# aleksandrina-streltsova/lidar-global-registration

Hardware: AMD Instinct MI355X
Metric: scan-pair registrations/sec (higher is better)
Workload: dtype f32

## Files before the change

### lidar-global-registration_amd/csrc/lgr_match.hip

```cpp
#include <rocprim/device/device_radix_sort.hpp>
#include <rocprim/device/device_scan.hpp>

#include <algorithm>
#include <vector>

#include "lgr_internal.h"

#include "lgr_match_common.cuh"
#include "lgr_match_cluster.cuh"
#include "lgr_match_pack.cuh"
#include "lgr_match_mfma.cuh"
#include "lgr_match_sweep.cuh"
#include "lgr_match_bounds.cuh"
#include "lgr_match_rerank.cuh"

extern "C" int lgr_match_last_stats(lgr_ctx* ctx, unsigned* out6) {
    if (!ctx || !out6) return LGR_ERR_INVALID_ARG;
    const lgr_match_stats& s = ctx->mstats;
    out6[0] = s.items_ab; out6[1] = s.dense_ab; out6[2] = s.items_ba;
    out6[3] = s.dense_ba; out6[4] = (unsigned) s.sub_cols; out6[5] = (unsigned) s.rg_rows;
    return LGR_OK;
}
extern "C" int lgr_match_last_work(lgr_ctx* ctx, double* executed_fraction) {
    if (!ctx || !executed_fraction) return LGR_ERR_INVALID_ARG;
// ... 136 lines not shown
struct MatchPrep {
    bool armed = false;
    const float* d_a = nullptr;
    int ma = 0, mb = 0;
    bool both = false;
    lgr_match_options mopt{};
    int sub = 1, rg_rows = BLOCK_ROWS, ns = 0;
    float *cen = nullptr, *cen2 = nullptr, *smp = nullptr, *basis = nullptr;
    int* smp_ok = nullptr;
    IrrRef* irr = nullptr;
    bool basis_ready = false;
    Side A;
};
static void match_prep_free(void* p) { delete (MatchPrep*) p; }
static MatchPrep* match_prep_of(lgr_ctx* ctx) {
    if (!ctx->match_prep) { ctx->match_prep = new MatchPrep(); ctx->match_prep_free = match_prep_free; }
    return (MatchPrep*) ctx->match_prep;
}

static int match_cluster(lgr_ctx* ctx, const float* d_a, int ma, const float* d_b, int mb, bool both, bool basis_side_by_side, MatchPrep* P) {
    const lgr_match_options& mo = ctx->mopt;
    int sub = 1;
    while (sub < SUBMAX && (long long) KCL * sub * 1024 < std::max(ma, mb)) sub *= 2;
    if (mo.leaves > 0) sub = mo.leaves;
    sub = std::min(SUBMAX, std::max(1, sub));
    const int n_leaves = KCL * sub;
    const int ns = 2 * KM_SAMPLE;
    char* misc;
    Carve carve{8192};
    const size_t o_cen2 = carve((size_t) MAXLEAF * 33 * 4);
    const size_t o_smp = carve((size_t) ns * 33 * 4), o_ok = carve((size_t) ns * 4), o_label = carve((size_t) ns * 4);
    const size_t o_cbuf = carve((size_t) 2 * KCL * 33 * 4), o_basis = carve((size_t) (34 * 33 + 64) * 4);
    const size_t o_skeys = carve((size_t) 2 * ns * 4), o_svals = carve((size_t) ns * 4), o_sidx = carve((size_t) ns * 4), o_coff = carve(256);
    const size_t o_zero = carve.off;
    const size_t o_kmax = carve(256), o_irr = carve(sizeof(IrrRef)), o_acc1 = carve((size_t) KM_ITERS * KCL * sizeof(KmAcc)), o_acc2 = carve((size_t) MAXLEAF * sizeof(KmAcc));
    const size_t zero_bytes = carve.off - o_zero;
    LGR_TRY(lgr_ws_t(ctx, WS_MATCH_MISC, carve.off, &misc));
    float* cen = (float*) (misc + 256);
    float* cen2 = (float*) (misc + o_cen2);
    float* smp = (float*) (misc + o_smp);
    int* smp_ok = (int*) (misc + o_ok);
    int* label = (int*) (misc + o_label);
    float* cbuf = (float*) (misc + o_cbuf);
    float* basis = (float*) (misc + o_basis);
    unsigned* skeys = (unsigned*) (misc + o_skeys);
    int* svals = (int*) (misc + o_svals);
    int* sidx = (int*) (misc + o_sidx);
    int* coff = (int*) (misc + o_coff);
    unsigned* kmax = (unsigned*) (misc + o_kmax);
    KmAcc* acc1 = (KmAcc*) (misc + o_acc1);
    KmAcc* acc2 = (KmAcc*) (misc + o_acc2);
    LGR_HIP(ctx, hipMemsetAsync(misc + o_zero, 0, zero_bytes, ctx->stream));
    IrrRef* irr = mo.irregular_rows ? (IrrRef*) (misc + o_irr) : nullptr;
    if (irr) km_consensus<<<cdiv(ns, 256), 256, 0, ctx->stream>>>(d_a, ma, d_b, mb, KM_SAMPLE, irr);
    km_sample<<<cdiv(ns, 256), 256, 0, ctx->stream>>>(d_a, ma, d_b, mb, KM_SAMPLE, smp, smp_ok, kmax, irr);
    auto lloyd = [&](lgr_ctx* cx) -> int {
        km_init<<<1, 64, 0, cx->stream>>>(smp, smp_ok, ns, cbuf);
        for (int it = 0; it <= KM_ITERS; ++it) {
            const bool last = it == KM_ITERS;
            km1_step<<<cdiv(ns, KM1_THREADS), KM1_THREADS, 0, cx->stream>>>(smp, smp_ok, ns, kmax, cbuf + (it & 1) * KCL * 33, it ? acc1 + (size_t) (it - 1) * KCL : nullptr,
                                                                            last ? nullptr : acc1 + (size_t) it * KCL, last ? cen : cbuf + ((it + 1) & 1) * KCL * 33, label);
        }
        km_label_keys<<<cdiv(ns, 256), 256, 0, cx->stream>>>(label, ns, skeys, svals);
        LGR_TRY(lgr_sort_pairs_u32(cx, skeys, skeys + ns, svals, sidx, (size_t) ns, 0, 5));
        km_cluster_offsets<<<1, 64, 0, cx->stream>>>(skeys + ns, ns, coff);
        km2_init<<<KCL, 64, 0, cx->stream>>>(smp, sidx, coff, cen, sub, cen2);
        if (sub > 1) {
            for (int it = 0; it < KM2_ITERS; ++it) {
                km2_step<<<dim3(KM2_PIECES, KCL), KM2_THREADS, 0, cx->stream>>>(smp, sidx, coff, kmax, cen2, sub, acc2);
                km2_finalize<<<n_leaves, 64, 0, cx->stream>>>(acc2, kmax, cen2);
            }
        }
        LGR_HIP(cx, hipGetLastError());
        return LGR_OK;
    };
    const bool want_basis = mo.box_bounds != 0;
    if (want_basis && basis_side_by_side) {
        LGR_TRY(lgr_run_pair(ctx, lloyd, [&](lgr_ctx* cx) { return box_basis(cx, mo.box_bounds == 2, smp, smp_ok, ns, basis, []() { return (int) LGR_OK; }); }));
    } else if (want_basis) {
        LGR_TRY(box_basis(ctx, mo.box_bounds == 2, smp, smp_ok, ns, basis, [&]() { return lloyd(ctx); }));
    } else {
        LGR_TRY(lloyd(ctx));
    }
    auto pick_group = [](size_t q_count, size_t t_count) {
        int g = 1024;
        while (g < 4096 && (t_count / g + 1) * q_count * 4 > ((size_t) 6 << 30)) g *= 2;
        return g;
    };
    int rg_rows = both ? pick_group((size_t) mb, (size_t) ma) : BLOCK_ROWS;
    if (ma <= 65536) rg_rows = BLOCK_ROWS;
    P->d_a = d_a; P->ma = ma; P->mb = mb; P->both = both; P->mopt = mo;
    P->sub = sub; P->rg_rows = rg_rows; P->ns = ns;
    P->cen = cen; P->cen2 = cen2; P->smp = smp; P->smp_ok = smp_ok; P->basis = basis; P->basis_ready = want_basis; P->irr = irr;
    return LGR_OK;
}

int lgr_match_prepare(lgr_ctx* ctx, const float* d_a, int ma, int mb, bool both) {
    MatchPrep* P = match_prep_of(ctx);
    P->armed = false;
    if (!d_a || ma <= 0 || mb <= 0) return LGR_OK;
    LGR_HIP(ctx, hipSetDevice(ctx->device));
    LGR_TRY(match_cluster(ctx, d_a, ma, nullptr, mb, both, false, P));
    P->armed = true;
    return LGR_OK;
}
void lgr_match_prepare_cancel(lgr_ctx* ctx) {
    if (ctx && ctx->match_prep) ((MatchPrep*) ctx->match_prep)->armed = false;
// ... 283 lines not shown
    if (f16 && env_int("LGR_MATCH_DEBUG", 0))
        fprintf(stderr, "[lgr] operand statistics: max |x - c|^2 %.6g, dropped energy %.6g (A %.6g, B %.6g) -> %s; irregular rows %d + %d\n", (double) r2, (double) drop2,
                (double) A.nstat_drop, (double) B.nstat_drop, os.rot ? "rotated" : "plain", A.n_irr, B.n_irr);
    st.f16 = f16 ? (os.rot ? 2 : 1) : 0;
    KS = !f16 ? OpFmt<FMT_F32>::KS : os.rot ? OpFmt<FMT_F16R>::KS : OpFmt<FMT_F16>::KS;
    NF = !f16 ? OpFmt<FMT_F32>::NF : os.rot ? OpFmt<FMT_F16R>::NF : OpFmt<FMT_F16>::NF;
    const size_t frag_bytes = f16 ? sizeof(f16x8) : sizeof(float);
    const size_t a_op_bytes = (size_t) ta * NF * 64 * frag_bytes;
    bset_stride = (size_t) tb * NF * 64;
    LGR_TRY(lgr_ws_t(ctx, WS_MATCH_ROWMIN, a_op_bytes + 256, &Aop));
    const size_t b_op_bytes = KCL * bset_stride * frag_bytes;
    LGR_TRY(lgr_ws_t(ctx, WS_MATCH_COLMIN, b_op_bytes + 256, &Bop));
    n_rg = cdiv(ma_pad, rg_rows);
    return LGR_OK;
}

int MatchCall::upload_group_tables() {
    std::vector<int> h_group_start, h_tiles(2 * (size_t) tb);
    int group_cols = GROUP_COLS;
    while (group_cols < 65536 && ((size_t) mb_pad / group_cols + n_leaves) * (size_t) ma_pad * 4 > ((size_t) 24 << 30)) group_cols *= 2;
    for (int l = 0; l < n_leaves; ++l)
        for (int s0 = B.h_leaf_start[l]; s0 < B.h_leaf_start[l + 1]; s0 += group_cols) {
            int s1 = std::min(B.h_leaf_start[l + 1], s0 + group_cols), g = (int) h_group_start.size();
            h_group_start.push_back(s0);
            for (int t = s0 / TILE; t < s1 / TILE; ++t) { h_tiles[t] = g; h_tiles[tb + t] = l; }
        }
    n_groups = (int) h_group_start.size();
    st.sub_cols = n_groups;
    h_group_start.push_back(mb_pad);
    LGR_TRY(lgr_ws_t(ctx, WS_MATCH_BEST_B, (size_t) KCL * n_groups + 2 * (size_t) n_rg + 2 * (size_t) tb + 2 * (size_t) n_groups + n_leaves + 72, &gmaxB));
    gmaxA = gmaxB + (size_t) KCL * n_groups;
    cl_of_rg = (int*) (gmaxA + n_rg);
    tile_group = cl_of_rg + n_rg;
    tile_leaf = tile_group + tb;
    group_start = tile_leaf + tb;
    group_leaf = group_start + n_groups + 1;
    leaf_g0 = group_leaf + n_groups;
    std::vector<int> h(n_rg), hgl(n_groups), hl(n_leaves + 1, n_groups);
    for (int g = 0; g < n_rg; ++g) h[g] = A.h_blkcl[(size_t) g * (rg_rows / BLOCK_ROWS)];
    for (int g = 0; g < n_groups; ++g) hgl[g] = h_tiles[tb + h_group_start[g] / TILE];
    for (int g = n_groups - 1; g >= 0; --g) hl[hgl[g]] = g;
    for (int l = n_leaves - 1; l >= 0; --l) hl[l] = std::min(hl[l], hl[l + 1]);
    LGR_HIP(ctx, hipMemcpyAsync(cl_of_rg, h.data(), h.size() * 4, hipMemcpyHostToDevice, ctx->stream));
    LGR_HIP(ctx, hipMemcpyAsync(tile_group, h_tiles.data(), h_tiles.size() * 4, hipMemcpyHostToDevice, ctx->stream));
    LGR_HIP(ctx, hipMemcpyAsync(group_start, h_group_start.data(), h_group_start.size() * 4, hipMemcpyHostToDevice, ctx->stream));
    LGR_HIP(ctx, hipMemcpyAsync(group_leaf, hgl.data(), hgl.size() * 4, hipMemcpyHostToDevice, ctx->stream));
    LGR_HIP(ctx, hipMemcpyAsync(leaf_g0, hl.data(), hl.size() * 4, hipMemcpyHostToDevice, ctx->stream));
    LGR_HIP(ctx, hipStreamSynchronize(ctx->stream));
    return LGR_OK;
}

static void launch_pack16(bool rot, hipStream_t s, const float* X, const int* perm, int n_pad, int role, const float* cen, const int* blkcl, const F16Scale& sc,
                          void* op, float* nrm, float2* shell) {
    if (rot) pack16_kernel<true><<<cdiv(n_pad, 256), 256, 0, s>>>(X, perm, n_pad, role, cen, blkcl, sc, (_Float16*) op, nrm, shell);
    else pack16_kernel<false><<<cdiv(n_pad, 256), 256, 0, s>>>(X, perm, n_pad, role, cen, blkcl, sc, (_Float16*) op, nrm, shell);
}

PruneWs MatchCall::carve_prune_ws(char* base) const {
    Carve carve{0, base};
    PruneWs w{};
    const size_t n_pairs = (size_t) n_rb * n_leaves;
    w.LBsq = carve.take<float>(n_pairs * 4);
    w.done = carve.take<uint8_t>(n_pairs);
    w.sched = carve.take<uint8_t>(n_pairs);
    w.touched = carve.take<uint8_t>(n_pairs);
    w.mask = carve.take<unsigned>((size_t) n_rb * n_cc * 4);
    w.mask_acc = carve.take<unsigned>((size_t) n_rb * n_cc * 4);
    w.u_rb = carve.take<float>((size_t) n_rb * 4);
    w.u_rt = carve.take<float>((size_t) n_rb * (BLOCK_ROWS / TILE) * 4);
    w.u_leaf = carve.take<unsigned>((size_t) MAXLEAF * 4);
    w.stats = carve.take<MaskStats>(sizeof(MaskStats));
    w.lb_part = carve.take<uint2>((size_t) n_rb * sizeof(uint2));
    w.leaf_first = carve.take<int>((size_t) MAXLEAF * 4);
    w.leaf_last = carve.take<int>((size_t) MAXLEAF * 4);
    w.mask_chk = carve.take<unsigned>(mo.self_check ? (size_t) 2 * n_rb * n_cc * 4 + 256 : 0);
    w.u_stage = carve.take<unsigned>((size_t) n_stage_total * 4);
    w.u_ct = carve.take<unsigned>((size_t) tb * 4);
    w.comp_r = carve.take<uint8_t>((size_t) n_rb * n_groups);
    w.comp_c = carve.take<uint8_t>((size_t) n_leaves * n_rg);
    w.smaxB = carve.take<float>((size_t) KCL * n_stage_total * 4);
    w.coarse_cnt = carve.take<unsigned long long>(32);
    w.u_row = carve.take<float>((size_t) ma_pad * 4);
    w.u_colv = carve.take<float>((size_t) mb_pad * 4);
    w.stage_shell = carve.take<float2>((size_t) KCL * n_stage_total * 8);
    w.rb_shell = carve.take<float2>((size_t) n_rb * 8);
    w.cperm = carve.take<int>((size_t) (n_leaves + TILE) * 4);
    w.cnrm = carve.take<float>((size_t) KCL * (n_leaves + TILE) * 4);
    w.cop = carve.take<f16x8>((size_t) KCL * ((n_leaves + TILE) / TILE) * 7 * 64 * sizeof(f16x8));
    w.clear_begin = (char*) w.done; w.clear_end = (char*) w.comp_r;
    w.bytes = carve.off;
    return w;
}
int MatchCall::prepare_prune_ws() {
    hipStream_t s3 = ctx->stream;
    if (f16) LGR_TRY(lgr_ctx_stream3(ctx, &s3));
    sB.start(ctx, s3, ctx->ev3, s3 != ctx->stream);
    n_cc = cdiv(mb_pad, CHUNK_COLS);
    n_cpad = pad_to(n_leaves, TILE);
    cset_stride = (size_t) (n_cpad / TILE) * NF * 64;
    if (!prune) return LGR_OK;
    char* pb;
    LGR_TRY(lgr_ws_t(ctx, WS_MATCH_PRUNE, carve_prune_ws(nullptr).bytes, &pb));
    W = carve_prune_ws(pb);
    LGR_TRY(sB.fork(ctx->ev[31]));
    LGR_HIP(ctx, hipMemsetAsync(W.clear_begin, 0, W.clear_end - W.clear_begin, sB.s));
    if (f16) {
        centre_perm_kernel<<<cdiv(n_cpad, 256), 256, 0, sB.s>>>(n_leaves, n_cpad, W.cperm);
        launch_pack16(os.rot, sB.s, cen2, W.cperm, n_cpad, 1, cen, nullptr, os.sc, W.cop, W.cnrm, nullptr);
// ... 424 lines not shown
```

### lidar-global-registration_amd/csrc/lgr_match_cluster.cuh

```cuda
#pragma once
#include "lgr_match_common.cuh"

namespace {

struct KmAcc { long long sum[33]; long long cnt; };
__device__ __forceinline__ double km_scale(unsigned kmax_bits) {
    return kmax_bits ? ldexp(1.0, 40 - ((int) (kmax_bits >> 23) - 127)) : 1.0;
}
constexpr int IRR_CAND = 16;
constexpr int IRR_CAP = 1024;
struct IrrRef { double s[3]; double tol; int enabled; int best; unsigned n_ok; unsigned agree[IRR_CAND]; };
__device__ __forceinline__ void block_sums(const float* v, double& s0, double& s1, double& s2) {
    s0 = 0.0; s1 = 0.0; s2 = 0.0;
#pragma unroll
    for (int k = 0; k < 11; ++k) { s0 += (double) v[k]; s1 += (double) v[11 + k]; s2 += (double) v[22 + k]; }
}
__device__ __forceinline__ bool sums_agree(double a0, double a1, double a2, double r0, double r1, double r2, double tol) {
    return fabs(a0 - r0) <= tol && fabs(a1 - r1) <= tol && fabs(a2 - r2) <= tol;
}
__device__ __forceinline__ double sums_tol(double r0, double r1, double r2) { return 1e-5 * fmax(fmax(fabs(r0), fabs(r1)), fabs(r2)); }
__device__ __forceinline__ const float* sample_row(int s, const float* __restrict__ A, int ma, const float* __restrict__ B, int mb, int per_side) {
    const bool fromA = !B || s < per_side;
    const float* X = fromA ? A : B;
    const int m = fromA ? ma : mb;
    if (m <= 0) return nullptr;
    const int t = fromA ? s : s - per_side;
    const long long i = (long long) t * m / (B ? per_side : 2 * per_side);
    return X + (size_t) i * 33;
}
__device__ __forceinline__ bool irr_decide(const IrrRef* __restrict__ ref, int& best) {
    unsigned top = 0u;
    best = 0;
    for (int c = 0; c < IRR_CAND; ++c) { const unsigned a = ref->agree[c]; if (a > top) { top = a; best = c; } }
    const unsigned n_ok = ref->n_ok;
    return n_ok >= 256u && (unsigned long long) top * 1000ull >= (unsigned long long) n_ok * 995ull;
}
__global__ __launch_bounds__(256) void km_consensus(const float* __restrict__ A, int ma, const float* __restrict__ B, int mb, int per_side, IrrRef* __restrict__ ref) {
    __shared__ double cs[IRR_CAND][3];
    __shared__ int cok[IRR_CAND];
    const int ns = 2 * per_side;
    if (threadIdx.x < IRR_CAND) {
        const float* r = sample_row((int) ((long long) threadIdx.x * ns / IRR_CAND), A, ma, B, mb, per_side);
        float v[33];
        const bool ok = r && row_finite(r, v);
        double s0 = 0.0, s1 = 0.0, s2 = 0.0;
        if (ok) block_sums(v, s0, s1, s2);
        cs[threadIdx.x][0] = s0; cs[threadIdx.x][1] = s1; cs[threadIdx.x][2] = s2;
        cok[threadIdx.x] = ok ? 1 : 0;
    }
    __syncthreads();
    const int s = blockIdx.x * blockDim.x + threadIdx.x;
    bool ok = false;
    double s0 = 0.0, s1 = 0.0, s2 = 0.0;
    if (s < ns) {
        const float* r = sample_row(s, A, ma, B, mb, per_side);
        float v[33];
        ok = r && row_finite(r, v);
        if (ok) block_sums(v, s0, s1, s2);
    }
    const int lane = threadIdx.x & 63;
    for (int c = 0; c < IRR_CAND; ++c) {
        const bool a = ok && cok[c] && sums_agree(s0, s1, s2, cs[c][0], cs[c][1], cs[c][2], sums_tol(cs[c][0], cs[c][1], cs[c][2]));
        const int n = __popcll(__ballot(a));
        if (lane == 0 && n) atomicAdd(&ref->agree[c], (unsigned) n);
    }
    const int n_ok = __popcll(__ballot(ok));
    if (lane == 0 && n_ok) atomicAdd(&ref->n_ok, (unsigned) n_ok);
}
__global__ void km_sample(const float* __restrict__ A, int ma, const float* __restrict__ B, int mb, int per_side,
                          float* __restrict__ smp, int* __restrict__ smp_ok, unsigned* __restrict__ kmax , IrrRef* __restrict__ irr_ref) {
    int s = blockIdx.x * blockDim.x + threadIdx.x;
    if (s >= 2 * per_side) return;
    const float* r = sample_row(s, A, ma, B, mb, per_side);
    float v[33];
    bool ok = r && row_finite(r, v);
    if (irr_ref) {
        int best;
        const bool on = irr_decide(irr_ref, best);
        double r0 = 0.0, r1 = 0.0, r2 = 0.0;
        if (on) {
            const float* rr = sample_row((int) ((long long) best * (2 * per_side) / IRR_CAND), A, ma, B, mb, per_side);
            float w[33];
            (void) row_finite(rr, w);
            block_sums(w, r0, r1, r2);
            if (ok) {
                double s0, s1, s2;
                block_sums(v, s0, s1, s2);
                ok = sums_agree(s0, s1, s2, r0, r1, r2, sums_tol(r0, r1, r2));
            }
        }
        if (s == 0) { irr_ref->s[0] = r0; irr_ref->s[1] = r1; irr_ref->s[2] = r2; irr_ref->tol = sums_tol(r0, r1, r2); irr_ref->best = best; irr_ref->enabled = on ? 1 : 0; }
    }
    float mx = 0.f;
    for (int k = 0; k < 33; ++k) { smp[(size_t) s * 33 + k] = ok ? v[k] : 0.f; if (ok) mx = fmaxf(mx, fabsf(v[k])); }
    smp_ok[s] = ok ? 1 : 0;
    for (int o = 32; o > 0; o >>= 1) mx = fmaxf(mx, __shfl_xor(mx, o));
    if ((threadIdx.x & 63) == 0 && mx > 0.f) atomicMax(kmax, __float_as_uint(mx));
}
__global__ void km_init(const float* __restrict__ smp, const int* __restrict__ smp_ok, int ns, float* __restrict__ cen) {
    int c = threadIdx.x;
    if (c >= KCL) return;
    int s = (int) ((long long) c * ns / KCL);
    int tries = 0;
    while (!smp_ok[s] && tries < ns) { s = (s + 1) % ns; ++tries; }
    for (int k = 0; k < 33; ++k) cen[c * 33 + k] = smp_ok[s] ? smp[(size_t) s * 33 + k] : 0.f;
}
__device__ __forceinline__ int nearest_centre(const float* v, const float* __restrict__ cen, float& best) {
    int bi = 0;
    best = __uint_as_float(0x7f800000u);
#pragma unroll 1
    for (int c = 0; c < KCL; ++c) {
        float d = 0.f;
#pragma unroll
        for (int k = 0; k < 33; ++k) { float t = v[k] - cen[c * 33 + k]; d = d + t * t; }
        if (d < best) { best = d; bi = c; }
    }
    return bi;
}
constexpr int KM1_THREADS = 256;
__global__ __launch_bounds__(KM1_THREADS) void km1_step(const float* __restrict__ smp, const int* __restrict__ smp_ok, int ns, const unsigned* __restrict__ kmax,
// ... 10 lines not shown
        if (blockIdx.x == 0) cen_out[e] = v;
    }
    for (int e = threadIdx.x; e < KCL * 34; e += KM1_THREADS) acc_s[e] = 0;
    __syncthreads();
    const int s = blockIdx.x * KM1_THREADS + threadIdx.x;
    if (s < ns) {
        int c = -1;
        if (smp_ok[s]) {
            float v[33], d;
#pragma unroll
            for (int k = 0; k < 33; ++k) v[k] = smp[(size_t) s * 33 + k];
            c = nearest_centre(v, cen_s, d);
            if (acc_out) {
#pragma unroll
                for (int k = 0; k < 33; ++k) atomicAdd((unsigned long long*) &acc_s[c * 34 + k], (unsigned long long) (long long) rint((double) v[k] * scale));
                atomicAdd((unsigned long long*) &acc_s[c * 34 + 33], 1ull);
            }
        }
        label[s] = c;
    }
    if (!acc_out) return;
    __syncthreads();
    long long* out = (long long*) acc_out;
    for (int e = threadIdx.x; e < KCL * 34; e += KM1_THREADS)
        if (acc_s[e] != 0) atomicAdd((unsigned long long*) &out[e], (unsigned long long) acc_s[e]);
}
__global__ void km_label_keys(const int* __restrict__ label, int ns, unsigned* __restrict__ keys, int* __restrict__ vals) {
    int s = blockIdx.x * blockDim.x + threadIdx.x;
    if (s >= ns) return;
    const int l = label[s];
    keys[s] = l < 0 ? (unsigned) KCL : (unsigned) l;
    vals[s] = s;
}
__global__ void km_cluster_offsets(const unsigned* __restrict__ keys_sorted, int ns, int* __restrict__ coff ) {
    const int p = threadIdx.x;
    if (p > KCL) return;
    int lo = 0, hi = ns;
    while (lo < hi) { const int mid = (lo + hi) >> 1; if (keys_sorted[mid] < (unsigned) p) lo = mid + 1; else hi = mid; }
    coff[p] = lo;
}
__global__ __launch_bounds__(64) void km2_init(const float* __restrict__ smp, const int* __restrict__ sidx, const int* __restrict__ coff,
                                               const float* __restrict__ cen, int sub, float* __restrict__ cen2) {
    const int p = blockIdx.x, lane = threadIdx.x;
    const int c0 = coff[p], cnt = coff[p + 1] - c0;
    for (int j = lane; j < sub; j += 64) {
        const float* src = cen + p * 33;
        if (cnt > 0) {
            const long long r = ((long long) j * cnt + sub - 1) / sub;
            if (r < cnt && (int) (r * sub / cnt) == j) src = smp + (size_t) sidx[c0 + (int) r] * 33;
        }
        for (int k = 0; k < 33; ++k) cen2[((size_t) p * sub + j) * 33 + k] = src[k];
    }
}
__device__ __forceinline__ int nearest_sub(const float* v, const float* __restrict__ c2 , int sub, float& best) {
    int bj = 0;
    best = __uint_as_float(0x7f800000u);
#pragma unroll 1
    for (int j = 0; j < sub; ++j) {
        float d = 0.f;
#pragma unroll
        for (int k = 0; k < 33; ++k) { float t = v[k] - c2[j * 33 + k]; d = d + t * t; }
        if (d < best) { best = d; bj = j; }
    }
    return bj;
}
constexpr int KM2_THREADS = 256, KM2_LANES = 4, KM2_SAMPLES = KM2_THREADS / KM2_LANES, KM2_PIECES = 48;
__global__ __launch_bounds__(KM2_THREADS) void km2_step(const float* __restrict__ smp, const int* __restrict__ sidx, const int* __restrict__ coff,
                                                        const unsigned* __restrict__ kmax, const float* __restrict__ cen2, int sub, KmAcc* __restrict__ acc2) {
    __shared__ float c2s[SUBMAX * 33];
    __shared__ long long acc_s[SUBMAX * 34];
    const int p = blockIdx.y;
    const int c0 = coff[p], s1 = coff[p + 1];
    if (c0 + (int) blockIdx.x * KM2_SAMPLES >= s1) return;
    for (int e = threadIdx.x; e < sub * 33; e += KM2_THREADS) c2s[e] = cen2[(size_t) p * sub * 33 + e];
    for (int e = threadIdx.x; e < sub * 34; e += KM2_THREADS) acc_s[e] = 0;
    __syncthreads();
    const double scale = km_scale(*kmax);
    const int q = threadIdx.x & (KM2_LANES - 1);
    for (int s0 = c0 + blockIdx.x * KM2_SAMPLES; s0 < s1; s0 += gridDim.x * KM2_SAMPLES) {
        const int s = s0 + (threadIdx.x >> 2);
        const bool act = s < s1;
        float v[33];
        const float* row = smp + (size_t) sidx[act ? s : s1 - 1] * 33;
#pragma unroll
        for (int k = 0; k < 33; ++k) v[k] = row[k];
        float best = __uint_as_float(0x7f800000u);
        int bj = 0x7fffffff;
#pragma unroll 1
        for (int j = q; j < sub; j += KM2_LANES) {
            float d = 0.f;
#pragma unroll
            for (int k = 0; k < 33; ++k) { float t = v[k] - c2s[j * 33 + k]; d = d + t * t; }
            if (d < best) { best = d; bj = j; }
        }
#pragma unroll
        for (int o = 1; o < KM2_LANES; o <<= 1) {
            const float ob = __shfl_xor(best, o);
            const int oj = __shfl_xor(bj, o);
            if (ob < best || (ob == best && oj < bj)) { best = ob; bj = oj; }
        }
        if (bj == 0x7fffffff) bj = 0;
        if (act) {
#pragma unroll
            for (int k = 0; k < 33; ++k)
                if ((k & (KM2_LANES - 1)) == q) atomicAdd((unsigned long long*) &acc_s[bj * 34 + k], (unsigned long long) (long long) rint((double) v[k] * scale));
            if (q == 1) atomicAdd((unsigned long long*) &acc_s[bj * 34 + 33], 1ull);
        }
    }
    __syncthreads();
    long long* out = (long long*) (acc2 + (size_t) p * sub);
    for (int e = threadIdx.x; e < sub * 34; e += KM2_THREADS)
        if (acc_s[e] != 0) atomicAdd((unsigned long long*) &out[e], (unsigned long long) acc_s[e]);
}
__global__ __launch_bounds__(64) void km2_finalize(KmAcc* __restrict__ acc2, const unsigned* __restrict__ kmax, float* __restrict__ cen2) {
    const int leaf = blockIdx.x, k = threadIdx.x;
    const long long cnt = acc2[leaf].cnt;
    __syncthreads();
    if (k < 33) {
        if (cnt > 0) cen2[(size_t) leaf * 33 + k] = (float) (((double) acc2[leaf].sum[k] / km_scale(*kmax)) / (double) cnt);
        acc2[leaf].sum[k] = 0;
    } else if (k == 33) acc2[leaf].cnt = 0;
}

constexpr int ASSIGN_THREADS = 1024;
__global__ __launch_bounds__(ASSIGN_THREADS) void assign_kernel(const float* __restrict__ X, int m, const float* __restrict__ cen, const float* __restrict__ cen2, int sub,
                                                                unsigned* __restrict__ keys, int* __restrict__ vals, uint8_t* __restrict__ valid,
                                                                int* __restrict__ counts , unsigned* __restrict__ rmax ,
                                                                int role, unsigned* __restrict__ nstat ,
                                                                const IrrRef* __restrict__ irr_ref , int* __restrict__ irr_list ) {
    extern __shared__ float c2s[];
    const int pitch = sub * 33 + 1;
    int* lc = (int*) (c2s + KCL * pitch);
    unsigned* lr = (unsigned*) (lc + MAXLEAF + 1);
    for (int e = threadIdx.x; e < KCL * sub * 33; e += blockDim.x) c2s[(e / (sub * 33)) * pitch + e % (sub * 33)] = cen2[e];
    for (int i = threadIdx.x; i <= MAXLEAF; i += blockDim.x) { lc[i] = 0; if (i < MAXLEAF) lr[i] = 0u; }
    __shared__ double cs_s[KCL][3];
    if (threadIdx.x < KCL * 3) {
        const int cc = threadIdx.x / 3, j = threadIdx.x % 3;
        double t = 0.0;
        for (int k = 0; k < 11; ++k) t += (double) cen[cc * 33 + 11 * j + k];
        cs_s[cc][j] = t;
    }
    __syncthreads();
    int i = blockIdx.x * blockDim.x + threadIdx.x;
    float st_n2 = 0.f, st_drop = 0.f;
    bool st_ovf = false;
    if (i < m) {
        float v[33], r2;
        bool ok = row_finite(X + (size_t) i * 33, v);
        unsigned key = 0xffffffffu;
        bool irr = false;
        double bx0 = 0.0, bx1 = 0.0, bx2 = 0.0;
        if (ok) block_sums(v, bx0, bx1, bx2);
        if (ok && irr_ref && irr_ref->enabled) {
            irr = !sums_agree(bx0, bx1, bx2, irr_ref->s[0], irr_ref->s[1], irr_ref->s[2], irr_ref->tol);
            if (irr) {
                const unsigned pos = atomicAdd(&nstat[3], 1u);
                if (pos < (unsigned) IRR_CAP) irr_list[pos] = i;
            }
        }
        if (ok && !irr) {
            int c = 0;
            r2 = __uint_as_float(0x7f800000u);
            float own_drop = 0.f;
#pragma unroll 1
            for (int cc = 0; cc < KCL; ++cc) {
                float d = 0.f;
#pragma unroll
                for (int k = 0; k < 33; ++k) {
                    const float t = v[k] - cen[cc * 33 + k];
                    d = d + t * t;
                }
                const double mg = 6.6e-7 * (double) sqrtf(d);
                const double s0 = fabs(bx0 - cs_s[cc][0]) + mg, s1 = fabs(bx1 - cs_s[cc][1]) + mg, s2 = fabs(bx2 - cs_s[cc][2]) + mg;
                const float dr = (float) (((s0 * s0 + s1 * s1) + s2 * s2) * (1.0001 / 11.0)) * 1.000001f + 1e-20f * d;
                if (d < r2) { r2 = d; c = cc; own_drop = dr; }
                if (role == 1) {
                    if (d < FLT_BIG) st_n2 = fmaxf(st_n2, d); else st_ovf = true;
                    st_drop = fmaxf(st_drop, dr);
                }
            }
            if (role == 0) {
                if (r2 < FLT_BIG) st_n2 = r2; else st_ovf = true;
                st_drop = own_drop;
            }
            float rl2;
            int j = nearest_sub(v, c2s + c * pitch, sub, rl2);
            if (!(r2 < FLT_BIG)) r2 = __uint_as_float(0x7f800000u);
            if (!(rl2 < FLT_BIG)) rl2 = __uint_as_float(0x7f800000u);
            int leaf = c * sub + j;
            key = ((unsigned) leaf << 22) | (__float_as_uint(r2) >> 9);
            atomicAdd(&lc[leaf], 1);
            atomicMax(&lr[leaf], __float_as_uint(rl2));
        }
        if (!ok || irr) atomicAdd(&lc[MAXLEAF], 1);
        keys[i] = key; vals[i] = i; valid[i] = ok ? (irr ? 2 : 1) : 0;
    }
    __syncthreads();
    for (int l = threadIdx.x; l <= MAXLEAF; l += blockDim.x) {
        if (lc[l]) atomicAdd(&counts[l], lc[l]);
        if (l < MAXLEAF && lr[l]) atomicMax(&rmax[l], lr[l]);
    }
    for (int o = 32; o > 0; o >>= 1) { st_n2 = fmaxf(st_n2, __shfl_xor(st_n2, o)); st_drop = fmaxf(st_drop, __shfl_xor(st_drop, o)); }
    const bool any_ovf = __ballot(st_ovf) != 0ull;
    if ((threadIdx.x & 63) == 0) {
        if (st_n2 > 0.f && __float_as_uint(st_n2) > *(volatile unsigned*) &nstat[0]) atomicMax(&nstat[0], __float_as_uint(st_n2));
        if (st_drop > 0.f && __float_as_uint(st_drop) > *(volatile unsigned*) &nstat[1]) atomicMax(&nstat[1], __float_as_uint(st_drop));
        if (any_ovf) nstat[2] = 1u;
    }
}

__global__ void place_kernel(const unsigned* __restrict__ keys_sorted, const int* __restrict__ vals_sorted, int n_valid,
                             const int* __restrict__ sorted_start , const int* __restrict__ pad_start ,
                             int* __restrict__ perm) {
    int s = blockIdx.x * blockDim.x + threadIdx.x;
    if (s >= n_valid) return;
    int l = (int) (keys_sorted[s] >> 22);
    perm[pad_start[l] + (s - sorted_start[l])] = vals_sorted[s];
}


}
```

### lidar-global-registration_amd/csrc/lgr_match_pack.cuh

```cuda
#pragma once
#include "lgr_match_common.cuh"

namespace {

__global__ void pack_kernel(const float* __restrict__ X, const int* __restrict__ perm, int n_pad, int role,
                            const float* __restrict__ cen, const int* __restrict__ blkcl,
                            float* __restrict__ P, float* __restrict__ nrm, unsigned* __restrict__ ovf) {
    int pos = blockIdx.x * blockDim.x + threadIdx.x;
    if (pos >= n_pad) return;
    int set = role == 1 ? blockIdx.y : 0;
    int o = perm[pos];
    int c = role == 1 ? set : blkcl[pos / BLOCK_ROWS];
    float v[33];
    float n2 = 0.f;
    if (o >= 0) {
#pragma unroll
        for (int k = 0; k < 33; ++k) { v[k] = X[(size_t) o * 33 + k] - cen[c * 33 + k]; n2 = n2 + v[k] * v[k]; }
    } else {
#pragma unroll
        for (int k = 0; k < 33; ++k) v[k] = 0.f;
        n2 = __uint_as_float(0x7f800000u);
    }
    nrm[(size_t) set * n_pad + pos] = n2;
    if (o >= 0 && !(n2 < FLT_BIG)) *ovf = 1u;
    int tile = pos >> 5, r = pos & 31;
    float* base = P + ((size_t) set * (n_pad / TILE) + tile) * KK * 64 + r;
#pragma unroll
    for (int k = 0; k < 34; ++k) {
        float val;
        if (k < 33) val = role == 0 ? -2.0f * v[k] : v[k];
        else val = role == 0 ? 1.0f : n2;
        base[(k >> 1) * 64 + (k & 1) * 32] = val;
    }
}

__device__ __forceinline__ void helmert11(const float* __restrict__ x, float* __restrict__ y, float* u) {
    const float rs[10] = {0.70710678118654752f, 0.40824829046386302f, 0.28867513459481288f, 0.22360679774997897f, 0.18257418583505537f,
                          0.15430334996209191f, 0.13363062095621219f, 0.11785113019775793f, 0.10540925533894598f, 0.09534625892455924f};
    float pre = x[0];
#pragma unroll
    for (int k = 1; k <= 10; ++k) {
        y[k - 1] = (pre - (float) k * x[k]) * rs[k - 1];
        pre = pre + x[k];
    }
    *u = pre * 0.30151134457776363f;
}

template <bool ROT>
__global__ __launch_bounds__(256) void pack16_kernel(const float* __restrict__ X, const int* __restrict__ perm, int n_pad, int role,
                              const float* __restrict__ cen, const int* __restrict__ blkcl, F16Scale sc,
                              _Float16* __restrict__ P, float* __restrict__ nrm, float2* __restrict__ shell ) {
    int pos = blockIdx.x * blockDim.x + threadIdx.x;
    const bool in_range = pos < n_pad;
    if (!in_range) pos = n_pad - 1;
    const int n_sets = role == 1 ? KCL : 1;
    const int o = perm[pos];
    float x0[33];
#pragma unroll
    for (int k = 0; k < 33; ++k) x0[k] = o >= 0 ? X[(size_t) o * 33 + k] : 0.f;
#pragma unroll 1
    for (int set = 0; set < n_sets; ++set) {
    const int c = role == 1 ? set : blkcl[pos / BLOCK_ROWS];
    float v[33];
    float n2 = 0.f;
    if (o >= 0) {
#pragma unroll
        for (int k = 0; k < 33; ++k) { v[k] = x0[k] - cen[c * 33 + k]; n2 = n2 + v[k] * v[k]; }
    } else {
#pragma unroll
        for (int k = 0; k < 33; ++k) v[k] = 0.f;
        n2 = __uint_as_float(0x7f800000u);
    }
    if (in_range) nrm[(size_t) set * n_pad + pos] = n2;
    if (shell) {
        const bool fin = in_range && n2 < FLT_BIG;
        float mn = fin ? n2 : __uint_as_float(0x7f800000u), mx = fin ? n2 : 0.f;
#pragma unroll
        for (int o = 16; o > 0; o >>= 1) { mn = fminf(mn, __shfl_xor(mn, o)); mx = fmaxf(mx, __shfl_xor(mx, o)); }
        if (in_range && (pos & 31) == 0)
            shell[(size_t) set * (n_pad / TILE) + (pos >> 5)] = make_float2(mn < FLT_BIG ? sqrtf(mn) * 0.9999998f : mn, sqrtf(mx) * 1.0000002f);
    }
    float y[30], u0, u1, u2;
    if (ROT) { helmert11(v, y, &u0); helmert11(v + 11, y + 10, &u1); helmert11(v + 22, y + 20, &u2); }
    if (!in_range) continue;
    constexpr int nd = ROT ? 30 : 33, nf = ROT ? OpFmt<FMT_F16R>::NF : OpFmt<FMT_F16>::NF;
    int tile = pos >> 5, r = pos & 31;
    _Float16 hv[nf * 16];
    auto put = [&](int cidx, _Float16 h) { hv[cidx] = h; };
    const float mul = role == 0 ? -2.0f * sc.s_mul : sc.s_mul;
    float n2m = n2;
    if (ROT && o >= 0) {
        n2m = 0.f;
#pragma unroll
        for (int k = 0; k < 30; ++k) n2m = n2m + y[k] * y[k];
    }
    constexpr int o12 = ROT ? 32 : nd, o21 = ROT ? 32 : 2 * nd;
#pragma unroll
    for (int k = 0; k < nd; ++k) {
        float x = (ROT ? y[k] : v[k]) * mul;
        _Float16 h1 = (_Float16) x;
        _Float16 h2 = (_Float16) (x - (float) h1);
        if (ROT) { put(k, h1); put(o12 + k, h2); }
        else if (role == 0) { put(k, h1); put(o12 + k, h1); put(o21 + k, h2); }
        else { put(k, h1); put(o12 + k, h2); put(o21 + k, h1); }
    }
    const bool rows = role == 0;
    const _Float16 c0 = (_Float16) sc.a_norm[0], c1 = (_Float16) sc.a_norm[1], c2 = (_Float16) sc.a_norm[2];
    const float N = n2m * (sc.s_mul * sc.s_mul);
    if (ROT) {
        _Float16 n1 = (_Float16) 65504.f, n2 = (_Float16) __uint_as_float(0x7f800000u);
        if (o >= 0 && N / sc.a_norm[0] < 65504.f) {
            n1 = (_Float16) (N / sc.a_norm[0]);
// ... 76 lines not shown
```

### lidar-global-registration_amd/csrc/lgr_match_rerank.cuh

```cuda
#pragma once
#include "lgr_match_common.cuh"
#include "lgr_match_cluster.cuh"

namespace {

__device__ __forceinline__ float exact_l2(const float* __restrict__ a, const float* __restrict__ b) {
    float acc[4][4];
#pragma unroll
    for (int i = 0; i < 4; ++i)
#pragma unroll
        for (int l = 0; l < 4; ++l) acc[i][l] = 0.f;
#pragma unroll
    for (int blk = 0; blk < 2; ++blk)
#pragma unroll
        for (int i = 0; i < 4; ++i)
#pragma unroll
            for (int l = 0; l < 4; ++l) {
                int j = 16 * blk + 4 * i + l;
                float t = a[j] - b[j];
                acc[i][l] = t * t + acc[i][l];
            }
    float s[4];
#pragma unroll
    for (int l = 0; l < 4; ++l) s[l] = ((acc[0][l] + acc[1][l]) + acc[2][l]) + acc[3][l];
// ... 826 lines not shown
}

__global__ void fill_u64(unsigned long long* __restrict__ p, int n, unsigned long long v) {
    int i = blockIdx.x * blockDim.x + threadIdx.x;
    if (i < n) p[i] = v;
}

__global__ void rerank_finalize(const unsigned long long* __restrict__ best, int nq, int block, int nblocks,
                                int32_t* __restrict__ idx, float* __restrict__ dist) {
    int i = blockIdx.x * blockDim.x + threadIdx.x;
    if (i >= nq) return;
    unsigned long long k = best[i];
    if (k == ~0ull) { idx[i] = -1; dist[i] = 0.f; return; }
    unsigned rank = (unsigned) (k & 0xffffffffu);
    int qb = rank / block, r = rank % block;
    int blk = nblocks - 1 - qb;
    idx[i] = blk * block + r;
    dist[i] = __uint_as_float((unsigned) (k >> 32));
}

int pad_to(int v, int m) { return (v + m - 1) / m * m; }

struct Side {
    int m = 0, n_valid = 0, n_pad = 0;
    int* perm = nullptr;
    uint8_t* valid = nullptr;
    int* blkcl = nullptr;
    int* leaf_start = nullptr;
    int* leaf_count = nullptr;
    unsigned* r2max = nullptr;
    float nstat_n2 = 0.f, nstat_drop = 0.f;
    bool nstat_ovf = false;
    int n_irr = 0;
    int* irr_list = nullptr;
    std::vector<int> h_blkcl;
    std::vector<int> h_leaf_start;
};

int build_side(lgr_ctx* ctx, const float* d_x, int m, const float* cen, const float* cen2, int sub, int leaf_unit, int cluster_unit,
               int ws_keys, int ws_perm, int role, const IrrRef* irr_ref, Side* s) {
    s->m = m;
    const int n_leaves = KCL * sub;
    unsigned *keys, *keys2;
    int *vals, *vals2;
    char* kbuf;
    size_t body = (((size_t) m * 17 + 255) & ~(size_t) 255);
    LGR_TRY(lgr_ws_t(ctx, ws_keys, body + 16384 + (size_t) IRR_CAP * 4, &kbuf));
    keys = (unsigned*) kbuf; keys2 = keys + m; vals = (int*) (keys2 + m); vals2 = vals + m;
    s->valid = (uint8_t*) (vals2 + m);
    int* counts = (int*) (kbuf + body);
    unsigned* rmax = (unsigned*) (kbuf + body + 8192);
    s->leaf_count = counts; s->r2max = rmax;
    LGR_HIP(ctx, hipMemsetAsync(counts, 0, 16384, ctx->stream));
    const size_t assign_lds = ((size_t) KCL * (sub * 33 + 1) + 2 * MAXLEAF + 1) * 4;
    if (assign_lds > 64 * 1024) LGR_HIP(ctx, hipFuncSetAttribute((const void*) assign_kernel, hipFuncAttributeMaxDynamicSharedMemorySize, (int) assign_lds));
    unsigned* nstat = (unsigned*) (kbuf + body + 12288);
    s->irr_list = (int*) (kbuf + body + 16384);
    assign_kernel<<<cdiv(m, ASSIGN_THREADS), ASSIGN_THREADS, assign_lds, ctx->stream>>>(d_x, m, cen, cen2, sub, keys, vals, s->valid, counts, rmax, role, nstat, irr_ref, s->irr_list);
    LGR_TRY(lgr_sort_pairs_u32(ctx, keys, keys2, vals, vals2, (size_t) m, 0, 32));
    int* h;
    LGR_TRY(lgr_pinned(ctx, 8192, (void**) &h));
    LGR_HIP(ctx, hipMemcpyAsync(h, counts, (MAXLEAF + 1) * 4, hipMemcpyDeviceToHost, ctx->stream));
    LGR_HIP(ctx, hipMemcpyAsync(h + MAXLEAF + 8, nstat, 16, hipMemcpyDeviceToHost, ctx->stream));
    LGR_HIP(ctx, hipStreamSynchronize(ctx->stream));
    memcpy(&s->nstat_n2, h + MAXLEAF + 8, 4);
    memcpy(&s->nstat_drop, h + MAXLEAF + 9, 4);
    s->nstat_ovf = h[MAXLEAF + 10] != 0;
    s->n_irr = h[MAXLEAF + 11];
    std::vector<int> starts(2 * (size_t) MAXLEAF + 2, 0);
    int acc = 0, pacc = 0;
    s->h_blkcl.clear();
    s->h_leaf_start.assign(n_leaves + 1, 0);
    for (int c = 0; c < KCL; ++c) {
        int cluster_begin = pacc;
        for (int j = 0; j < sub; ++j) {
            int l = c * sub + j;
            starts[l] = acc; starts[MAXLEAF + l] = pacc;
            s->h_leaf_start[l] = pacc;
            acc += h[l];
            pacc += pad_to(h[l], leaf_unit);
        }
        pacc = pad_to(pacc, cluster_unit);
        for (int b = 0; b < (pacc - cluster_begin) / BLOCK_ROWS; ++b) s->h_blkcl.push_back(c);
    }
    s->h_leaf_start[n_leaves] = pacc;
    starts[MAXLEAF + n_leaves] = pacc;
    s->n_valid = acc; s->n_pad = pacc;
    if (s->n_pad == 0) return LGR_OK;
    int* pbuf;
    LGR_TRY(lgr_ws_t(ctx, ws_perm, (size_t) s->n_pad + s->h_blkcl.size() + starts.size() + 64, &pbuf));
    s->perm = pbuf; s->blkcl = pbuf + s->n_pad;
    int* d_starts = s->blkcl + s->h_blkcl.size();
    s->leaf_start = d_starts + MAXLEAF;
    LGR_HIP(ctx, hipMemsetAsync(s->perm, 0xff, (size_t) s->n_pad * 4, ctx->stream));
    LGR_HIP(ctx, hipMemcpyAsync(s->blkcl, s->h_blkcl.data(), s->h_blkcl.size() * 4, hipMemcpyHostToDevice, ctx->stream));
    LGR_HIP(ctx, hipMemcpyAsync(d_starts, starts.data(), starts.size() * 4, hipMemcpyHostToDevice, ctx->stream));
    LGR_HIP(ctx, hipStreamSynchronize(ctx->stream));
    if (s->n_valid) place_kernel<<<cdiv(s->n_valid, 256), 256, 0, ctx->stream>>>(keys2, vals2, s->n_valid, d_starts, d_starts + MAXLEAF, s->perm);
    return LGR_OK;
}

template <bool ROWDIR>
int run_rerank(lgr_ctx* ctx, EpsExtra ex, CompView comp, const float* table, int n_groups, int group_size, const int* starts, const float* Q, const Side& qs,
               const float* nQ, const float* nQ_sets, const float* gmax, const int* cl_of_group,
               const float* T, const float* Tsorted, const Side& ts, int block, unsigned long long* best, int32_t* d_idx, float* d_dist,
               unsigned* stat_items, unsigned* stat_dense, bool force_dense, RefilterArgs ra, unsigned* stat_pairs) {
    const int q_pad = qs.n_pad;
    unsigned* dense;
    LGR_TRY(lgr_ws_t(ctx, WS_MATCH_DENSE, (size_t) q_pad * (4 + CAND_KEEP) + 64, &dense));
    float* thr = (float*) (dense + q_pad);
    int* counts = (int*) (dense + 2 * (size_t) q_pad);
// ... 72 lines not shown
```

Measured before the change: 46.34.

## Rework clustering and packing kernels: per-wave consensus, paired sub-centroid LDS, coop row loads

Several preprocessing kernels change at once. km_consensus now has each 64-lane wave handle multiple rows, keeps the candidate sums in registers shared via shuffles, and accumulates agreement counts before issuing one atomic per wave instead of one per candidate per block. assign_kernel interleaves pairs of sub-centroids in LDS so two distances are computed with 2-wide vector math, loads rows with 16-byte reads, and runs as a grid-stride loop capped at the CU count so the centroid table is staged into LDS fewer times. pack16_kernel for role 0 loads rows cooperatively through LDS for coalesced global reads. The grid-stride change also alters how per-thread stats are reduced (now max), and the cooperative path adds a sync and 33 KB of LDS per block.

```diff
diff --git a/lidar-global-registration_amd/csrc/lgr_match.hip b/lidar-global-registration_amd/csrc/lgr_match.hip
--- a/lidar-global-registration_amd/csrc/lgr_match.hip
+++ b/lidar-global-registration_amd/csrc/lgr_match.hip
@@ -212,7 +212,7 @@
     KmAcc* acc2 = (KmAcc*) (misc + o_acc2);
     LGR_HIP(ctx, hipMemsetAsync(misc + o_zero, 0, zero_bytes, ctx->stream));
     IrrRef* irr = mo.irregular_rows ? (IrrRef*) (misc + o_irr) : nullptr;
-    if (irr) km_consensus<<<cdiv(ns, 256), 256, 0, ctx->stream>>>(d_a, ma, d_b, mb, KM_SAMPLE, irr);
+    if (irr) km_consensus<<<cdiv(ns, KMC_THREADS * KMC_ROWS), KMC_THREADS, 0, ctx->stream>>>(d_a, ma, d_b, mb, KM_SAMPLE, irr);
     km_sample<<<cdiv(ns, 256), 256, 0, ctx->stream>>>(d_a, ma, d_b, mb, KM_SAMPLE, smp, smp_ok, kmax, irr);
     auto lloyd = [&](lgr_ctx* cx) -> int {
         km_init<<<1, 64, 0, cx->stream>>>(smp, smp_ok, ns, cbuf);
@@ -602,8 +602,14 @@
 
 static void launch_pack16(bool rot, hipStream_t s, const float* X, const int* perm, int n_pad, int role, const float* cen, const int* blkcl, const F16Scale& sc,
                           void* op, float* nrm, float2* shell) {
-    if (rot) pack16_kernel<true><<<cdiv(n_pad, 256), 256, 0, s>>>(X, perm, n_pad, role, cen, blkcl, sc, (_Float16*) op, nrm, shell);
-    else pack16_kernel<false><<<cdiv(n_pad, 256), 256, 0, s>>>(X, perm, n_pad, role, cen, blkcl, sc, (_Float16*) op, nrm, shell);
+    const dim3 g(cdiv(n_pad, 256));
+    if (role == 0) {
+        if (rot) pack16_kernel<true, true><<<g, 256, 0, s>>>(X, perm, n_pad, role, cen, blkcl, sc, (_Float16*) op, nrm, shell);
+        else pack16_kernel<false, true><<<g, 256, 0, s>>>(X, perm, n_pad, role, cen, blkcl, sc, (_Float16*) op, nrm, shell);
+    } else {
+        if (rot) pack16_kernel<true, false><<<g, 256, 0, s>>>(X, perm, n_pad, role, cen, blkcl, sc, (_Float16*) op, nrm, shell);
+        else pack16_kernel<false, false><<<g, 256, 0, s>>>(X, perm, n_pad, role, cen, blkcl, sc, (_Float16*) op, nrm, shell);
+    }
 }
 
 PruneWs MatchCall::carve_prune_ws(char* base) const {
diff --git a/lidar-global-registration_amd/csrc/lgr_match_cluster.cuh b/lidar-global-registration_amd/csrc/lgr_match_cluster.cuh
--- a/lidar-global-registration_amd/csrc/lgr_match_cluster.cuh
+++ b/lidar-global-registration_amd/csrc/lgr_match_cluster.cuh
@@ -35,37 +35,49 @@
     const unsigned n_ok = ref->n_ok;
     return n_ok >= 256u && (unsigned long long) top * 1000ull >= (unsigned long long) n_ok * 995ull;
 }
-__global__ __launch_bounds__(256) void km_consensus(const float* __restrict__ A, int ma, const float* __restrict__ B, int mb, int per_side, IrrRef* __restrict__ ref) {
-    __shared__ double cs[IRR_CAND][3];
-    __shared__ int cok[IRR_CAND];
+constexpr int KMC_ROWS = 8, KMC_THREADS = 64;
+__global__ __launch_bounds__(KMC_THREADS) void km_consensus(const float* __restrict__ A, int ma, const float* __restrict__ B, int mb, int per_side, IrrRef* __restrict__ ref) {
     const int ns = 2 * per_side;
-    if (threadIdx.x < IRR_CAND) {
-        const float* r = sample_row((int) ((long long) threadIdx.x * ns / IRR_CAND), A, ma, B, mb, per_side);
+    const int lane = threadIdx.x & 63;
+    double c0 = 0.0, c1 = 0.0, c2 = 0.0;
+    bool cok = false;
+    if (lane < IRR_CAND) {
+        const float* r = sample_row((int) ((long long) lane * ns / IRR_CAND), A, ma, B, mb, per_side);
         float v[33];
-        const bool ok = r && row_finite(r, v);
+        cok = r && row_finite(r, v);
+        if (cok) block_sums(v, c0, c1, c2);
+    }
+    const double ctol = sums_tol(c0, c1, c2);
+    const unsigned long long cok_mask = __ballot(cok);
+    const int wave = (blockIdx.x * KMC_THREADS + threadIdx.x) >> 6;
+    unsigned n_agree[IRR_CAND], n_ok = 0u;
+#pragma unroll
+    for (int c = 0; c < IRR_CAND; ++c) n_agree[c] = 0u;
+#pragma unroll 1
+    for (int it = 0; it < KMC_ROWS; ++it) {
+        const int s = (wave * KMC_ROWS + it) * 64 + lane;
+        bool ok = false;
         double s0 = 0.0, s1 = 0.0, s2 = 0.0;
-        if (ok) block_sums(v, s0, s1, s2);
-        cs[threadIdx.x][0] = s0; cs[threadIdx.x][1] = s1; cs[threadIdx.x][2] = s2;
-        cok[threadIdx.x] = ok ? 1 : 0;
-    }
-    __syncthreads();
-    const int s = blockIdx.x * blockDim.x + threadIdx.x;
-    bool ok = false;
-    double s0 = 0.0, s1 = 0.0, s2 = 0.0;
-    if (s < ns) {
-        const float* r = sample_row(s, A, ma, B, mb, per_side);
-        float v[33];
-        ok = r && row_finite(r, v);
-        if (ok) block_sums(v, s0, s1, s2);
-    }
-    const int lane = threadIdx.x & 63;
-    for (int c = 0; c < IRR_CAND; ++c) {
-        const bool a = ok && cok[c] && sums_agree(s0, s1, s2, cs[c][0], cs[c][1], cs[c][2], sums_tol(cs[c][0], cs[c][1], cs[c][2]));
-        const int n = __popcll(__ballot(a));
-        if (lane == 0 && n) atomicAdd(&ref->agree[c], (unsigned) n);
-    }
-    const int n_ok = __popcll(__ballot(ok));
-    if (lane == 0 && n_ok) atomicAdd(&ref->n_ok, (unsigned) n_ok);
+        if (s < ns) {
+            const float* r = sample_row(s, A, ma, B, mb, per_side);
+            float v[33];
+            ok = r && row_finite(r, v);
+            if (ok) block_sums(v, s0, s1, s2);
+        }
+#pragma unroll
+        for (int c = 0; c < IRR_CAND; ++c) {
+            const double r0 = __shfl(c0, c), r1 = __shfl(c1, c), r2 = __shfl(c2, c), tol = __shfl(ctol, c);
+            const bool a = ok && ((cok_mask >> c) & 1ull) && sums_agree(s0, s1, s2, r0, r1, r2, tol);
+            n_agree[c] += (unsigned) __popcll(__ballot(a));
+        }
+        n_ok += (unsigned) __popcll(__ballot(ok));
+    }
+    if (lane == 0) {
+#pragma unroll
+        for (int c = 0; c < IRR_CAND; ++c)
+            if (n_agree[c]) atomicAdd(&ref->agree[c], n_agree[c]);
+        if (n_ok) atomicAdd(&ref->n_ok, n_ok);
+    }
 }
 __global__ void km_sample(const float* __restrict__ A, int ma, const float* __restrict__ B, int mb, int per_side,
                           float* __restrict__ smp, int* __restrict__ smp_ok, unsigned* __restrict__ kmax , IrrRef* __restrict__ irr_ref) {
@@ -182,18 +194,6 @@
         for (int k = 0; k < 33; ++k) cen2[((size_t) p * sub + j) * 33 + k] = src[k];
     }
 }
-__device__ __forceinline__ int nearest_sub(const float* v, const float* __restrict__ c2 , int sub, float& best) {
-    int bj = 0;
-    best = __uint_as_float(0x7f800000u);
-#pragma unroll 1
-    for (int j = 0; j < sub; ++j) {
-        float d = 0.f;
-#pragma unroll
-        for (int k = 0; k < 33; ++k) { float t = v[k] - c2[j * 33 + k]; d = d + t * t; }
-        if (d < best) { best = d; bj = j; }
-    }
-    return bj;
-}
 constexpr int KM2_THREADS = 256, KM2_LANES = 4, KM2_SAMPLES = KM2_THREADS / KM2_LANES, KM2_PIECES = 48;
 __global__ __launch_bounds__(KM2_THREADS) void km2_step(const float* __restrict__ smp, const int* __restrict__ sidx, const int* __restrict__ coff,
                                                         const unsigned* __restrict__ kmax, const float* __restrict__ cen2, int sub, KmAcc* __restrict__ acc2) {
@@ -253,16 +253,62 @@
 }
 
 constexpr int ASSIGN_THREADS = 1024;
+constexpr int ASSIGN_PAIR = 72;
+__host__ __device__ constexpr int assign_pitch(int sub) { return ((((sub + 1) >> 1) * ASSIGN_PAIR + 63) & ~63) + 4; }
+__device__ __forceinline__ int assign_slot(int e ) { const int j = e / 33; return (j >> 1) * ASSIGN_PAIR + 2 * (e - j * 33) + (j & 1); }
+typedef float f32x2 __attribute__((ext_vector_type(2)));
+struct __attribute__((packed, aligned(4))) RowQuad { float x, y, z, w; };
+__device__ __forceinline__ bool row_finite16(const float* __restrict__ r, float* v) {
+#pragma unroll
+    for (int q = 0; q < 8; ++q) { const RowQuad w = *(const RowQuad*) (r + 4 * q); v[4 * q] = w.x; v[4 * q + 1] = w.y; v[4 * q + 2] = w.z; v[4 * q + 3] = w.w; }
+    v[32] = r[32];
+    bool ok = true;
+#pragma unroll
+    for (int k = 0; k < 33; ++k) ok = ok && (fabsf(v[k]) <= FLT_BIG);
+    return ok;
+}
+__device__ __forceinline__ int nearest_sub(const float* v, const float* c2 , int sub, float& best) {
+    int bj = 0;
+    best = __uint_as_float(0x7f800000u);
+#pragma unroll 1
+    for (int j = 0; j < sub; j += 2) {
+        const float4* row = (const float4*) (c2 + (j >> 1) * ASSIGN_PAIR);
+        f32x2 c[34];
+#pragma unroll
+        for (int q = 0; q < 17; ++q) { const float4 w = row[q]; c[2 * q] = f32x2{w.x, w.y}; c[2 * q + 1] = f32x2{w.z, w.w}; }
+        f32x2 d = {0.f, 0.f};
+#pragma unroll
+        for (int k = 0; k < 33; ++k) { const f32x2 t = f32x2{v[k], v[k]} - c[k]; d = d + t * t; }
+        if (d.x < best) { best = d.x; bj = j; }
+        if (j + 1 < sub && d.y < best) { best = d.y; bj = j + 1; }
+    }
+    return bj;
+}
 __global__ __launch_bounds__(ASSIGN_THREADS) void assign_kernel(const float* __restrict__ X, int m, const float* __restrict__ cen, const float* __restrict__ cen2, int sub,
                                                                 unsigned* __restrict__ keys, int* __restrict__ vals, uint8_t* __restrict__ valid,
                                                                 int* __restrict__ counts , unsigned* __restrict__ rmax ,
                                                                 int role, unsigned* __restrict__ nstat ,
                                                                 const IrrRef* __restrict__ irr_ref , int* __restrict__ irr_list ) {
-    extern __shared__ float c2s[];
-    const int pitch = sub * 33 + 1;
+    extern __shared__ __align__(16) float c2s[];
+    const int pitch = assign_pitch(sub);
     int* lc = (int*) (c2s + KCL * pitch);
     unsigned* lr = (unsigned*) (lc + MAXLEAF + 1);
-    for (int e = threadIdx.x; e < KCL * sub * 33; e += blockDim.x) c2s[(e / (sub * 33)) * pitch + e % (sub * 33)] = cen2[e];
+    const int n_el = sub * 33, lane = threadIdx.x & 63;
+    const bool vec = (sub & 3) == 0 && ((size_t) cen2 & 15) == 0;
+    for (int c = threadIdx.x >> 6; c < KCL; c += blockDim.x >> 6) {
+        const float* src = cen2 + (size_t) c * n_el;
+        float* dst = c2s + c * pitch;
+        if (vec) {
+            for (int e4 = lane; e4 < n_el / 4; e4 += 64) {
+                const float4 w = ((const float4*) src)[e4];
+                const float wv[4] = {w.x, w.y, w.z, w.w};
+#pragma unroll
+                for (int t = 0; t < 4; ++t) dst[assign_slot(4 * e4 + t)] = wv[t];
+            }
+        } else {
+            for (int e = lane; e < n_el; e += 64) dst[assign_slot(e)] = src[e];
+        }
+    }
     for (int i = threadIdx.x; i <= MAXLEAF; i += blockDim.x) { lc[i] = 0; if (i < MAXLEAF) lr[i] = 0u; }
     __shared__ double cs_s[KCL][3];
     if (threadIdx.x < KCL * 3) {
@@ -272,12 +318,12 @@
         cs_s[cc][j] = t;
     }
     __syncthreads();
-    int i = blockIdx.x * blockDim.x + threadIdx.x;
     float st_n2 = 0.f, st_drop = 0.f;
     bool st_ovf = false;
-    if (i < m) {
+#pragma unroll 1
+    for (int i = blockIdx.x * blockDim.x + threadIdx.x; i < m; i += gridDim.x * blockDim.x) {
         float v[33], r2;
-        bool ok = row_finite(X + (size_t) i * 33, v);
+        bool ok = row_finite16(X + (size_t) i * 33, v);
         unsigned key = 0xffffffffu;
         bool irr = false;
         double bx0 = 0.0, bx1 = 0.0, bx2 = 0.0;
@@ -311,8 +357,8 @@
                 }
             }
             if (role == 0) {
-                if (r2 < FLT_BIG) st_n2 = r2; else st_ovf = true;
-                st_drop = own_drop;
+                if (r2 < FLT_BIG) st_n2 = fmaxf(st_n2, r2); else st_ovf = true;
+                st_drop = fmaxf(st_drop, own_drop);
             }
             float rl2;
             int j = nearest_sub(v, c2s + c * pitch, sub, rl2);
diff --git a/lidar-global-registration_amd/csrc/lgr_match_pack.cuh b/lidar-global-registration_amd/csrc/lgr_match_pack.cuh
--- a/lidar-global-registration_amd/csrc/lgr_match_pack.cuh
+++ b/lidar-global-registration_amd/csrc/lgr_match_pack.cuh
@@ -46,7 +46,7 @@
     *u = pre * 0.30151134457776363f;
 }
 
-template <bool ROT>
+template <bool ROT, bool COOP>
 __global__ __launch_bounds__(256) void pack16_kernel(const float* __restrict__ X, const int* __restrict__ perm, int n_pad, int role,
                               const float* __restrict__ cen, const int* __restrict__ blkcl, F16Scale sc,
                               _Float16* __restrict__ P, float* __restrict__ nrm, float2* __restrict__ shell ) {
@@ -56,8 +56,23 @@
     const int n_sets = role == 1 ? KCL : 1;
     const int o = perm[pos];
     float x0[33];
-#pragma unroll
-    for (int k = 0; k < 33; ++k) x0[k] = o >= 0 ? X[(size_t) o * 33 + k] : 0.f;
+    if constexpr (COOP) {
+        __shared__ float rows_s[256 * 33];
+        float* ws = rows_s + (threadIdx.x >> 6) * (64 * 33);
+        const int lane = threadIdx.x & 63;
+#pragma unroll
+        for (int i = 0; i < 33; ++i) {
+            const int e = i * 64 + lane, row = e / 33, k = e - row * 33;
+            const int orow = __shfl(o, row);
+            ws[e] = orow >= 0 ? X[(size_t) orow * 33 + k] : 0.f;
+        }
+        __syncthreads();
+#pragma unroll
+        for (int k = 0; k < 33; ++k) x0[k] = ws[lane * 33 + k];
+    } else {
+#pragma unroll
+        for (int k = 0; k < 33; ++k) x0[k] = o >= 0 ? X[(size_t) o * 33 + k] : 0.f;
+    }
 #pragma unroll 1
     for (int set = 0; set < n_sets; ++set) {
     const int c = role == 1 ? set : blkcl[pos / BLOCK_ROWS];
diff --git a/lidar-global-registration_amd/csrc/lgr_match_rerank.cuh b/lidar-global-registration_amd/csrc/lgr_match_rerank.cuh
--- a/lidar-global-registration_amd/csrc/lgr_match_rerank.cuh
+++ b/lidar-global-registration_amd/csrc/lgr_match_rerank.cuh
@@ -902,11 +902,12 @@
     unsigned* rmax = (unsigned*) (kbuf + body + 8192);
     s->leaf_count = counts; s->r2max = rmax;
     LGR_HIP(ctx, hipMemsetAsync(counts, 0, 16384, ctx->stream));
-    const size_t assign_lds = ((size_t) KCL * (sub * 33 + 1) + 2 * MAXLEAF + 1) * 4;
+    const size_t assign_lds = ((size_t) KCL * assign_pitch(sub) + 2 * MAXLEAF + 1) * 4;
+    const int assign_grid = std::min(cdiv(m, ASSIGN_THREADS), std::max(1, ctx->n_cu));
     if (assign_lds > 64 * 1024) LGR_HIP(ctx, hipFuncSetAttribute((const void*) assign_kernel, hipFuncAttributeMaxDynamicSharedMemorySize, (int) assign_lds));
     unsigned* nstat = (unsigned*) (kbuf + body + 12288);
     s->irr_list = (int*) (kbuf + body + 16384);
-    assign_kernel<<<cdiv(m, ASSIGN_THREADS), ASSIGN_THREADS, assign_lds, ctx->stream>>>(d_x, m, cen, cen2, sub, keys, vals, s->valid, counts, rmax, role, nstat, irr_ref, s->irr_list);
+    assign_kernel<<<assign_grid, ASSIGN_THREADS, assign_lds, ctx->stream>>>(d_x, m, cen, cen2, sub, keys, vals, s->valid, counts, rmax, role, nstat, irr_ref, s->irr_list);
     LGR_TRY(lgr_sort_pairs_u32(ctx, keys, keys2, vals, vals2, (size_t) m, 0, 32));
     int* h;
     LGR_TRY(lgr_pinned(ctx, 8192, (void**) &h));
```

Result: no change. 46.80, median of 6 (+1.0%).
